# arcee-ai/DALM

Hardware: NVIDIA H100
Metric: RAG-e2e train-step samples/sec (bge-large + Llama-2-7B, bs=18) (higher is better)
Workload: dtype bf16

## Files before the change

dalm_b200/csrc/common.cuh:

```cuda
#pragma once
#include <cuda_runtime.h>
#include <cuda_bf16.h>
#include <stdint.h>
#include <stdio.h>
#include <string.h>

struct CUtensorMap_st;

namespace dalm {

void set_error(const char* fmt, ...);
int  check_launch(const char* what);
void count_launch(int n = 1);

#define DALM_REQUIRE(cond, ...)                                   \
  do {                                                            \
    if (!(cond)) { ::dalm::set_error(__VA_ARGS__); return 1; }    \
  } while (0)

#define DALM_CUDA(expr)                                                                   \
  do {                                                                                    \
    cudaError_t _e = (expr);                                                              \
    if (_e != cudaSuccess) {                                                              \
      ::dalm::set_error("%s failed: %s (%s:%d)", #expr, cudaGetErrorString(_e), __FILE__, \
                        __LINE__);                                                        \
      return 2;                                                                           \
    }                                                                                     \
  } while (0)

int num_sms();
long long l2_bytes();

int get_tmap(const void* ptr, long long rows, long long cols, long long ld, int box_rows, ::CUtensorMap_st* out, int f32 = 0);

__device__ __forceinline__ float warp_sum(float v) {
#pragma unroll
  for (int o = 16; o > 0; o >>= 1) v += __shfl_xor_sync(0xffffffffu, v, o);
  return v;
}
__device__ __forceinline__ float warp_max(float v) {
#pragma unroll
  for (int o = 16; o > 0; o >>= 1) v = fmaxf(v, __shfl_xor_sync(0xffffffffu, v, o));
  return v;
}
__device__ __forceinline__ double warp_sum_d(double v) {
#pragma unroll
  for (int o = 16; o > 0; o >>= 1) v += __shfl_xor_sync(0xffffffffu, v, o);
  return v;
}

__device__ __forceinline__ float block_sum(float v, float* red) {
  const int lane = threadIdx.x & 31, wid = threadIdx.x >> 5, nw = (blockDim.x + 31) >> 5;
  v = warp_sum(v);
  __syncthreads();
  if (lane == 0) red[wid] = v;
  __syncthreads();
  float r = (lane < nw) ? red[lane] : 0.f;
  r = warp_sum(r);
  return r;
}
__device__ __forceinline__ float block_max(float v, float* red) {
  const int lane = threadIdx.x & 31, wid = threadIdx.x >> 5, nw = (blockDim.x + 31) >> 5;
  v = warp_max(v);
  __syncthreads();
  if (lane == 0) red[wid] = v;
  __syncthreads();
  float r = (lane < nw) ? red[lane] : -INFINITY;
  r = warp_max(r);
  return r;
}

struct __align__(16) bf16x8 { __nv_bfloat162 v[4]; };

__device__ __forceinline__ void unpack8(const bf16x8& p, float* f) {
#pragma unroll
  for (int i = 0; i < 4; ++i) {
    float2 t = __bfloat1622float2(p.v[i]);
    f[2 * i] = t.x; f[2 * i + 1] = t.y;
  }
}
__device__ __forceinline__ bf16x8 pack8(const float* f) {
  bf16x8 p;
#pragma unroll
  for (int i = 0; i < 4; ++i) p.v[i] = __floats2bfloat162_rn(f[2 * i], f[2 * i + 1]);
  return p;
}

__device__ __forceinline__ float gelu_erf(float x) {
  return 0.5f * x * (1.f + erff(x * 0.70710678118654752440f));
}
__device__ __forceinline__ float gelu_erf_grad(float x) {
  const float cdf = 0.5f * (1.f + erff(x * 0.70710678118654752440f));
  const float pdf = 0.39894228040143267794f * __expf(-0.5f * x * x);
  return cdf + x * pdf;
}


struct DropCfg {
  float p;
  float inv_keep;
  unsigned int thresh;
  unsigned long long seed, stream;
  const unsigned long long* offset;
};
inline DropCfg make_drop(float p, unsigned long long seed, unsigned long long stream, const void* offset) {
  DropCfg d;
  d.p = p;
  double t = (double)p * 65536.0 + 0.5;
  d.thresh = p > 0.f ? (t >= 65535.0 ? 65535u : (unsigned int)t) : 0u;
  d.inv_keep = p > 0.f ? (float)(1.0 / (1.0 - (double)d.thresh / 65536.0)) : 1.f;
  d.seed = seed; d.stream = stream; d.offset = (const unsigned long long*)offset;
  return d;
}
__device__ __forceinline__ uint4 philox4x32_7(uint2 key, uint4 c) {
#pragma unroll
  for (int r = 0; r < 7; ++r) {
    const unsigned int hi0 = __umulhi(0xD2511F53u, c.x), lo0 = 0xD2511F53u * c.x;
    const unsigned int hi1 = __umulhi(0xCD9E8D57u, c.z), lo1 = 0xCD9E8D57u * c.z;
    c = make_uint4(hi1 ^ c.y ^ key.x, lo1, hi0 ^ c.w ^ key.y, lo0);
    key.x += 0x9E3779B9u; key.y += 0xBB67AE85u;
  }
  return c;
}
__device__ __forceinline__ unsigned long long drop_stream(const DropCfg& d) {
  return d.stream + (d.offset ? (*d.offset) * 0x9E3779B97F4A7C15ull : 0ull);
}
__device__ __forceinline__ void drop_scale8(const DropCfg& d, unsigned long long stream, unsigned long long idx8, float* scale) {
  const uint4 r = philox4x32_7(make_uint2((unsigned int)d.seed, (unsigned int)(d.seed >> 32)),
                               make_uint4((unsigned int)idx8, (unsigned int)(idx8 >> 32), (unsigned int)stream,
                                          (unsigned int)(stream >> 32)));
  const unsigned int w[4] = {r.x, r.y, r.z, r.w};
#pragma unroll
  for (int j = 0; j < 4; ++j) {
    scale[2 * j]     = (w[j] & 0xFFFFu) >= d.thresh ? d.inv_keep : 0.f;
    scale[2 * j + 1] = (w[j] >> 16)     >= d.thresh ? d.inv_keep : 0.f;
  }
}
__device__ __forceinline__ float drop_scale1(const DropCfg& d, unsigned long long stream, unsigned long long idx) {
  float sc[8];
  drop_scale8(d, stream, idx >> 3, sc);
  float v = sc[0];
#pragma unroll
  for (int j = 1; j < 8; ++j) if ((idx & 7) == (unsigned long long)j) v = sc[j];
  return v;
}

}
```

dalm_b200/csrc/gemm_wgmma.cu:

```cuda
#include "common.cuh"
#include "ptx.cuh"
#include <cudaTypedefs.h>
#include <mutex>
#include <unordered_map>

namespace dalm {
using namespace ptx;

enum class Epi {
  Plain,
  SwiGLU,
  RoPE,
  GeluPair,
  NormRoPE,
};

struct GemmEpilogue {
  void* out;
  long long ldo;
  int out_f32;
  const float* bias;
  const void* resid;
  long long ldr;
  int resid_f32;
  int act;
  float alpha;
  int M, N, K;
  DropCfg drop;
  int group_m;
  const float* rope_cos; const float* rope_sin;
  int rope_L, rope_cols;
  const float* q_norm; const float* k_norm;
  int nq_heads;
  float norm_eps;
  float* norm_rstd; long long ld_rstd;
  int norm_pre;
  int l2_hints;
};

__device__ __forceinline__ void tile_coords(int tile, int num_m, int num_n, int gm, int& m_blk, int& n_blk) {
  if (gm <= 0) { m_blk = tile % num_m; n_blk = tile / num_m; return; }
  const int band_tiles = gm * num_n;
  const int band = tile / band_tiles;
  const int r = tile - band * band_tiles;
  const int m0 = band * gm;
  const int h = min(gm, num_m - m0);
  const int n = r / h;
  m_blk = m0 + (r - n * h);
  n_blk = (band & 1) ? (num_n - 1 - n) : n;
}

template <bool PRE = false>
__device__ __forceinline__ void epilogue_math(const GemmEpilogue& ep, const uint32_t* v, float* f, int row, int col0, bool row_ok,
                                              const float4* rpre = nullptr) {
  const int N = ep.N;
#pragma unroll
  for (int i = 0; i < 32; ++i) f[i] = __uint_as_float(v[i]) * ep.alpha;
  if (ep.bias) {
#pragma unroll
    for (int i = 0; i < 32; ++i) if (col0 + i < N) f[i] += __ldg(ep.bias + col0 + i);
  }
  if (ep.act == 1) {
#pragma unroll
    for (int i = 0; i < 32; ++i) f[i] = gelu_erf(f[i]);
  }
  if (ep.drop.p > 0.f) {
    const unsigned long long dstream = drop_stream(ep.drop);
    const unsigned long long base = ((unsigned long long)row * (unsigned long long)N + (unsigned long long)col0) >> 3;
#pragma unroll
    for (int g = 0; g < 4; ++g) {
      float sc[8];
      drop_scale8(ep.drop, dstream, base + g, sc);
#pragma unroll
      for (int j = 0; j < 8; ++j) f[g * 8 + j] *= sc[j];
    }
  }
  if constexpr (PRE) {
#pragma unroll
    for (int g = 0; g < 8; ++g) { f[g * 4 + 0] += rpre[g].x; f[g * 4 + 1] += rpre[g].y; f[g * 4 + 2] += rpre[g].z; f[g * 4 + 3] += rpre[g].w; }
  } else if (ep.resid && row_ok) {
    if (ep.resid_f32) {
      const float* r = reinterpret_cast<const float*>(ep.resid) + (size_t)row * ep.ldr + col0;
#pragma unroll
      for (int g = 0; g < 8; ++g) {
        if (col0 + g * 4 < N) {
          const float4 t = *reinterpret_cast<const float4*>(r + g * 4);
          f[g * 4 + 0] += t.x; f[g * 4 + 1] += t.y; f[g * 4 + 2] += t.z; f[g * 4 + 3] += t.w;
        }
      }
    } else {
      const __nv_bfloat16* r = reinterpret_cast<const __nv_bfloat16*>(ep.resid) + (size_t)row * ep.ldr + col0;
#pragma unroll
      for (int g = 0; g < 4; ++g) {
        if (col0 + g * 8 < N) {
          const bf16x8 t = *reinterpret_cast<const bf16x8*>(r + g * 8);
          float tf[8];
          unpack8(t, tf);
          if (ep.act == 2) {
#pragma unroll
            for (int i = 0; i < 8; ++i) f[g * 8 + i] = __bfloat162float(__float2bfloat16_rn(f[g * 8 + i])) * gelu_erf_grad(tf[i]);
          } else {
#pragma unroll
            for (int i = 0; i < 8; ++i) f[g * 8 + i] += tf[i];
          }
        }
      }
    }
  }
}

__device__ __forceinline__ void acc_ld32(const float* p, uint32_t* v) {
#pragma unroll
  for (int g = 0; g < 8; ++g) {
    const float4 t = *reinterpret_cast<const float4*>(p + g * 4);
    v[g * 4 + 0] = __float_as_uint(t.x); v[g * 4 + 1] = __float_as_uint(t.y);
    v[g * 4 + 2] = __float_as_uint(t.z); v[g * 4 + 3] = __float_as_uint(t.w);
  }
}

constexpr int kStageTileBytes = 128 * 128;
constexpr int kEpiGroups = 2;
constexpr int kGemmThreads = 128 + kEpiGroups * 128;
template <int BN, Epi EPI>
__device__ __forceinline__ void epilogue_drain_tile(const GemmEpilogue& ep, const CUtensorMap* tmap_out, const CUtensorMap* tmap_out2,
                                                    unsigned char* staging, int grp, const float* arow, int row_in_tile, int tile_row0,
                                                    int tile_col0) {
  static_assert(BN == 256 || EPI == Epi::Plain || EPI == Epi::GeluPair, "the SwiGLU and RoPE epilogues need 256-wide tiles");
  const int N = ep.N;
  const int row = tile_row0 + row_in_tile;
  const bool row_ok = row < ep.M;
  constexpr bool F32_OUT = EPI == Epi::Plain;
  const int sb_cols = (F32_OUT && ep.out_f32) ? 32 : 64;
  const bool issuer = (threadIdx.x == 128 + grp * 128);
  unsigned char* tile = staging + grp * kStageTileBytes;
  unsigned char* st = tile + row_in_tile * 128;
  const int sw = row_in_tile & 7;
  const bool rpf = F32_OUT && ep.out_f32 && ep.resid != nullptr && ep.resid_f32;
  float4 rnext[8];
  auto fetch_resid = [&](int cc) {
    const int cg0 = tile_col0 + cc;
    const float* r = reinterpret_cast<const float*>(ep.resid) + (size_t)row * ep.ldr + cg0;
#pragma unroll
    for (int g = 0; g < 8; ++g)
      rnext[g] = (row_ok && cc < BN && cg0 + g * 4 < N) ? *reinterpret_cast<const float4*>(r + g * 4) : make_float4(0.f, 0.f, 0.f, 0.f);
  };
  if (rpf) fetch_resid(grp * sb_cols);
#pragma unroll 1
  for (int c = grp * sb_cols; c < BN; c += kEpiGroups * sb_cols) {
    const int col0 = tile_col0 + c;
    if (col0 >= N) break;
    if (issuer) bulk_wait_read<0>();
    named_bar_sync(1 + grp, 128);
    if (F32_OUT && ep.out_f32) {
      uint32_t v[32]; float f[32];
      acc_ld32(arow + c, v);
      if (rpf) {
        epilogue_math<true>(ep, v, f, row, col0, row_ok, rnext);
        fetch_resid(c + kEpiGroups * sb_cols);
      } else {
        epilogue_math<false>(ep, v, f, row, col0, row_ok);
      }
#pragma unroll
      for (int g = 0; g < 8; ++g)
        *reinterpret_cast<float4*>(st + ((g ^ sw) << 4)) = make_float4(f[g * 4], f[g * 4 + 1], f[g * 4 + 2], f[g * 4 + 3]);
    } else if (EPI == Epi::RoPE && col0 < ep.rope_cols) {
      const bool second = ((col0 >> 6) & 1) != 0;
      const int cp = second ? c - 64 : c + 64;
      const int colp = tile_col0 + cp;
      const int pos = row_ok ? (row % ep.rope_L) : 0;
      const float* cs = ep.rope_cos + (size_t)pos * 64;
      const float* sn = ep.rope_sin + (size_t)pos * 64;
#pragma unroll
      for (int h = 0; h < 2; ++h) {
        uint32_t vo[32], vq[32]; float f[32];
        acc_ld32(arow + (c + h * 32), vo);
        acc_ld32(arow + (cp + h * 32), vq);
        float cc[32], ss[32];
#pragma unroll
        for (int i = 0; i < 32; i += 4) {
          *reinterpret_cast<float4*>(cc + i) = __ldg(reinterpret_cast<const float4*>(cs + h * 32 + i));
          *reinterpret_cast<float4*>(ss + i) = __ldg(reinterpret_cast<const float4*>(sn + h * 32 + i));
        }
#pragma unroll
        for (int i = 0; i < 32; ++i) {
          float own = __uint_as_float(vo[i]), oth = __uint_as_float(vq[i]);
          if (ep.bias) {
            own += __ldg(ep.bias + col0 + h * 32 + i);
            oth += __ldg(ep.bias + colp + h * 32 + i);
          }
          f[i] = second ? fmaf(own, cc[i], oth * ss[i]) : fmaf(own, cc[i], -oth * ss[i]);
        }
#pragma unroll
        for (int g = 0; g < 4; ++g)
          *reinterpret_cast<bf16x8*>(st + (((h * 4 + g) ^ sw) << 4)) = pack8(f + g * 8);
      }
    } else if (EPI == Epi::NormRoPE && col0 < ep.rope_cols) {
      const bool second = ((col0 >> 6) & 1) != 0;
      const int cp = second ? c - 64 : c + 64;
      const int colp = tile_col0 + cp;
      const int c1 = second ? cp : c;
      const int head = col0 >> 7;
      const float* nw = head < ep.nq_heads ? ep.q_norm : ep.k_norm;
      const int jo = second ? 64 : 0, jp = 64 - jo;
      float ss = 0.f;
#pragma unroll 1
      for (int h = 0; h < 4; ++h) {
        uint32_t v[32];
        acc_ld32(arow + (c1 + h * 32), v);
#pragma unroll
        for (int i = 0; i < 32; ++i) {
          float x = __uint_as_float(v[i]);
          if (ep.bias) x += __ldg(ep.bias + tile_col0 + c1 + h * 32 + i);
          ss = fmaf(x, x, ss);
        }
      }
      const float rstd = rsqrtf(ss * (1.f / 128.f) + ep.norm_eps);
      if (ep.norm_rstd && row_ok && !second) ep.norm_rstd[(size_t)row * ep.ld_rstd + head] = rstd;
      const int pos = row_ok ? (row % ep.rope_L) : 0;
      const float* cs = ep.rope_cos + (size_t)pos * 64;
      const float* sn = ep.rope_sin + (size_t)pos * 64;
#pragma unroll
      for (int h = 0; h < 2; ++h) {
        uint32_t vo[32], vq[32]; float f[32];
        acc_ld32(arow + (c + h * 32), vo);
        acc_ld32(arow + (cp + h * 32), vq);
        float cc[32], ss2[32];
#pragma unroll
        for (int i = 0; i < 32; i += 4) {
          *reinterpret_cast<float4*>(cc + i) = __ldg(reinterpret_cast<const float4*>(cs + h * 32 + i));
          *reinterpret_cast<float4*>(ss2 + i) = __ldg(reinterpret_cast<const float4*>(sn + h * 32 + i));
        }
#pragma unroll
        for (int i = 0; i < 32; ++i) {
          float own = __uint_as_float(vo[i]), oth = __uint_as_float(vq[i]);
          if (ep.bias) {
            own += __ldg(ep.bias + col0 + h * 32 + i);
            oth += __ldg(ep.bias + colp + h * 32 + i);
          }
          own = own * rstd * __ldg(nw + jo + h * 32 + i);
          oth = oth * rstd * __ldg(nw + jp + h * 32 + i);
          f[i] = second ? fmaf(own, cc[i], oth * ss2[i]) : fmaf(own, cc[i], -oth * ss2[i]);
        }
#pragma unroll
        for (int g = 0; g < 4; ++g)
          *reinterpret_cast<bf16x8*>(st + (((h * 4 + g) ^ sw) << 4)) = pack8(f + g * 8);
      }
      fence_proxy_async();
      named_bar_sync(1 + grp, 128);
      if (issuer) {
        if (ep.l2_hints & 4) tma_store_2d_hint(tmap_out, tile, col0, tile_row0, l2_policy_evict_first());
        else                 tma_store_2d(tmap_out, tile, col0, tile_row0);
        bulk_commit();
      }
      if (!ep.norm_pre) continue;
      if (issuer) bulk_wait_read<0>();
      named_bar_sync(1 + grp, 128);
#pragma unroll
      for (int h = 0; h < 2; ++h) {
        uint32_t v[32]; float f[32];
        acc_ld32(arow + (c + h * 32), v);
#pragma unroll
        for (int i = 0; i < 32; ++i) {
          f[i] = __uint_as_float(v[i]);
          if (ep.bias) f[i] += __ldg(ep.bias + col0 + h * 32 + i);
        }
#pragma unroll
        for (int g = 0; g < 4; ++g)
          *reinterpret_cast<bf16x8*>(st + (((h * 4 + g) ^ sw) << 4)) = pack8(f + g * 8);
      }
      fence_proxy_async();
      named_bar_sync(1 + grp, 128);
      if (issuer) {
        tma_store_2d(tmap_out2, tile, col0, tile_row0);
        bulk_commit();
      }
      continue;
    } else if (EPI == Epi::GeluPair) {
      bf16x8 pk[8];
#pragma unroll
      for (int h = 0; h < 2; ++h) {
        if (col0 + h * 32 < N) {
          uint32_t v[32]; float f[32];
          acc_ld32(arow + (c + h * 32), v);
          epilogue_math(ep, v, f, row, col0 + h * 32, row_ok);
#pragma unroll
          for (int g = 0; g < 4; ++g) pk[h * 4 + g] = pack8(f + g * 8);
        } else {
#pragma unroll
          for (int g = 0; g < 4; ++g) pk[h * 4 + g] = bf16x8{};
        }
      }
#pragma unroll
      for (int g = 0; g < 8; ++g) *reinterpret_cast<bf16x8*>(st + ((g ^ sw) << 4)) = pk[g];
      fence_proxy_async();
      named_bar_sync(1 + grp, 128);
      if (issuer) {
        if (ep.l2_hints & 4) tma_store_2d_hint(tmap_out, tile, col0, tile_row0, l2_policy_evict_first());
        else                 tma_store_2d(tmap_out, tile, col0, tile_row0);
        bulk_commit();
      }
#pragma unroll
      for (int g = 0; g < 8; ++g) {
        float x[8];
        unpack8(pk[g], x);
#pragma unroll
        for (int i = 0; i < 8; ++i) x[i] = gelu_erf(x[i]);
        pk[g] = pack8(x);
      }
      if (issuer) bulk_wait_read<0>();
      named_bar_sync(1 + grp, 128);
#pragma unroll
      for (int g = 0; g < 8; ++g) *reinterpret_cast<bf16x8*>(st + ((g ^ sw) << 4)) = pk[g];
      fence_proxy_async();
      named_bar_sync(1 + grp, 128);
      if (issuer) {
        tma_store_2d(tmap_out2, tile, col0, tile_row0);
        bulk_commit();
      }
      continue;
    } else {
#pragma unroll
      for (int h = 0; h < 2; ++h) {
        if (col0 + h * 32 < N) {
          uint32_t v[32]; float f[32];
          acc_ld32(arow + (c + h * 32), v);
          epilogue_math(ep, v, f, row, col0 + h * 32, row_ok);
#pragma unroll
          for (int g = 0; g < 4; ++g)
            *reinterpret_cast<bf16x8*>(st + (((h * 4 + g) ^ sw) << 4)) = pack8(f + g * 8);
        }
      }
    }
    fence_proxy_async();
    named_bar_sync(1 + grp, 128);
    if (issuer) {
      if (ep.l2_hints & 4) tma_store_2d_hint(tmap_out, tile, col0, tile_row0, l2_policy_evict_first());
      else                 tma_store_2d(tmap_out, tile, col0, tile_row0);
      bulk_commit();
    }
  }
  if constexpr (EPI == Epi::SwiGLU) {
    const int j = grp;
    const int acol0 = (tile_col0 >> 1) + j * 64;
    if (issuer) bulk_wait_read<0>();
    named_bar_sync(1 + grp, 128);
#pragma unroll
    for (int h = 0; h < 2; ++h) {
      uint32_t vg[32], vu[32]; float f[32];
      acc_ld32(arow + (j * 64 + h * 32), vg);
      acc_ld32(arow + (128 + j * 64 + h * 32), vu);
#pragma unroll
      for (int i = 0; i < 32; ++i) {
        const float g = __uint_as_float(vg[i]);
        f[i] = g / (1.f + __expf(-g)) * __uint_as_float(vu[i]);
      }
#pragma unroll
      for (int g4 = 0; g4 < 4; ++g4) *reinterpret_cast<bf16x8*>(st + (((h * 4 + g4) ^ sw) << 4)) = pack8(f + g4 * 8);
    }
    fence_proxy_async();
    named_bar_sync(1 + grp, 128);
    if (issuer) {
      if (ep.l2_hints & 4) tma_store_2d_hint(tmap_out2, tile, acol0, tile_row0, l2_policy_evict_first());
      else                 tma_store_2d(tmap_out2, tile, acol0, tile_row0);
      bulk_commit();
    }
  }
}

template <int BN> struct GemmCfg {
  static constexpr int BM = 128, BK = 64;
  static constexpr int A_BYTES = BM * BK * 2;
  static constexpr int B_BYTES = BN * BK * 2;
  static constexpr int STAGE_BYTES = A_BYTES + B_BYTES;
  static constexpr int STAGES = (BN == 256) ? 4 : (BN == 128 ? 6 : 8);
  static constexpr int ACC_LD = BN + 4;
  static constexpr int SMEM_BYTES = STAGES * STAGE_BYTES + 2 * kStageTileBytes + 1024  + 256 ;
  static_assert(BM * ACC_LD * 4 <= STAGES * STAGE_BYTES, "the accumulator tile reuses the stage ring");
  static_assert(SMEM_BYTES <= 232448, "exceeds 227 KB of shared memory per block");
};

template <int BN, int TA, int TB>
__device__ __forceinline__ void wgmma_tile(float* d, uint64_t da, uint64_t db, int scale_d) {
  if constexpr (BN == 256) wgmma_m64n256k16<TA, TB>(d, da, db, scale_d);
  else if constexpr (BN == 128) wgmma_m64n128k16<TA, TB>(d, da, db, scale_d);
  else wgmma_m64n64k16<TA, TB>(d, da, db, scale_d);
}

template <int BN, int LAYOUT, Epi EPI, int CL>
__global__ void __launch_bounds__(kGemmThreads, 1)
gemm_bf16_tn_kernel(const __grid_constant__ CUtensorMap tmap_a, const __grid_constant__ CUtensorMap tmap_b,
                    const __grid_constant__ CUtensorMap tmap_out, const __grid_constant__ CUtensorMap tmap_out2, const GemmEpilogue ep) {
  using Cfg = GemmCfg<BN>;
  constexpr int BM = Cfg::BM, BK = Cfg::BK, STAGES = Cfg::STAGES;
  static_assert(CL == 1 || (LAYOUT == 0 && EPI == Epi::Plain), "the cluster kernel takes the plain TN layout");
  extern __shared__ unsigned char smem_raw[];
  unsigned char* smem = reinterpret_cast<unsigned char*>((reinterpret_cast<uintptr_t>(smem_raw) + 1023) & ~uintptr_t(1023));
  unsigned char* staging = smem + STAGES * Cfg::STAGE_BYTES;
  uint64_t* full_bar  = reinterpret_cast<uint64_t*>(staging + 2 * kStageTileBytes);
  uint64_t* empty_bar = full_bar + STAGES;
  uint64_t* epi_bar   = empty_bar + STAGES;
  float* acc_smem = reinterpret_cast<float*>(smem);

  const int warp = threadIdx.x >> 5, lane = threadIdx.x & 31;
  const uint32_t rank = CL == 2 ? cluster_ctarank() : 0u;
  const int M = ep.M, N = ep.N, K = ep.K;
  const int num_m = (M + CL * BM - 1) / (CL * BM), num_n = (N + BN - 1) / BN;
  const int num_tiles = num_m * num_n;
  const int num_kb = (K + BK - 1) / BK;
  const int unit = blockIdx.x / CL, num_units = gridDim.x / CL;
  const int group_m = CL == 2 ? 0 : ep.group_m;

  if (threadIdx.x == 0) {
    prefetch_tmap(&tmap_a);
    prefetch_tmap(&tmap_b);
    prefetch_tmap(&tmap_out);
    if constexpr (EPI == Epi::SwiGLU || EPI == Epi::GeluPair || EPI == Epi::NormRoPE) prefetch_tmap(&tmap_out2);
  }
  if (threadIdx.x == 32) {
    for (int s = 0; s < STAGES; ++s) { mbar_init(&full_bar[s], 1); mbar_init(&empty_bar[s], 8 * CL); }
    mbar_init(epi_bar, 8 * CL);
    fence_mbar_init();
  }
  if constexpr (CL == 2) cluster_sync_all();
  else __syncthreads();

  if (warp < 4) {
    asm volatile("setmaxnreg.dec.sync.aligned.u32 40;" ::: "memory");
    if (warp == 0 && lane == 0) {
      int stage = 0; uint32_t phase = 0;
      const bool hint_a = (ep.l2_hints & 1) != 0, hint_b = (ep.l2_hints & 2) != 0;
      const uint64_t pol_a = hint_a ? l2_policy_evict_last() : 0ull, pol_b = hint_b ? l2_policy_evict_first() : 0ull;
      auto load = [](void* dst, const CUtensorMap* tm, uint64_t* bar, int c0, int c1, bool hinted, uint64_t pol) {
        if (hinted) tma_load_2d_hint(dst, tm, bar, c0, c1, pol);
        else        tma_load_2d(dst, tm, bar, c0, c1);
      };
      int it = 0;
      for (int tile = unit; tile < num_tiles; tile += num_units, ++it) {
        int m_blk, n_blk;
        tile_coords(tile, num_m, num_n, group_m, m_blk, n_blk);
        if (it > 0) mbar_wait(epi_bar, (uint32_t)(it - 1) & 1u);
        for (int kb = 0; kb < num_kb; ++kb) {
          mbar_wait(&empty_bar[stage], phase ^ 1);
          unsigned char* sa = smem + stage * Cfg::STAGE_BYTES;
          unsigned char* sb = sa + Cfg::A_BYTES;
          mbar_arrive_expect_tx(&full_bar[stage], Cfg::STAGE_BYTES);
          if constexpr (CL == 2) {
            load(sa, &tmap_a, &full_bar[stage], kb * BK, (m_blk * CL + (int)rank) * BM, hint_a, pol_a);
            tma_load_2d_multicast(sb + rank * (Cfg::B_BYTES / 2), &tmap_b, &full_bar[stage], kb * BK, n_blk * BN + (int)rank * (BN / 2), 0x3);
          } else {
            if constexpr (LAYOUT == 2) {
#pragma unroll
              for (int c = 0; c < BM / 64; ++c) load(sa + c * 8192, &tmap_a, &full_bar[stage], m_blk * BM + c * 64, kb * BK, hint_a, pol_a);
            } else {
              load(sa, &tmap_a, &full_bar[stage], kb * BK, m_blk * BM, hint_a, pol_a);
            }
            if constexpr (LAYOUT >= 1) {
#pragma unroll
              for (int c = 0; c < BN / 64; ++c) load(sb + c * 8192, &tmap_b, &full_bar[stage], n_blk * BN + c * 64, kb * BK, hint_b, pol_b);
            } else {
              load(sb, &tmap_b, &full_bar[stage], kb * BK, n_blk * BN, hint_b, pol_b);
            }
          }
          if (++stage == STAGES) { stage = 0; phase ^= 1; }
        }
      }
    }
  } else {
    asm volatile("setmaxnreg.inc.sync.aligned.u32 232;" ::: "memory");
    const int grp = (warp - 4) >> 2;
    const int q = warp & 3;
    constexpr int TA = LAYOUT == 2 ? 1 : 0, TB = LAYOUT >= 1 ? 1 : 0;
    constexpr uint64_t a_step = TA ? 128 : 2, b_step = TB ? 128 : 2;
    const uint32_t a_off = (uint32_t)grp * 8192u;
    int stage = 0; uint32_t phase = 0;
    for (int tile = unit; tile < num_tiles; tile += num_units) {
      int m_blk, n_blk;
      tile_coords(tile, num_m, num_n, group_m, m_blk, n_blk);
      float acc[BN / 2];
      int prev = -1;
      for (int kb = 0; kb < num_kb; ++kb) {
        mbar_wait(&full_bar[stage], phase);
        const uint32_t sa = smem_u32(smem + stage * Cfg::STAGE_BYTES);
        const uint32_t sb = sa + Cfg::A_BYTES;
        const uint64_t adesc = TA ? make_sw128_mnmajor_desc(sa + a_off, 8192, 1024) : make_sw128_kmajor_desc(sa + a_off);
        const uint64_t bdesc = TB ? make_sw128_mnmajor_desc(sb, 8192, 1024) : make_sw128_kmajor_desc(sb);
        wgmma_fence();
#pragma unroll
        for (int k = 0; k < BK / 16; ++k)
          wgmma_tile<BN, TA, TB>(acc, adesc + a_step * (uint64_t)k, bdesc + b_step * (uint64_t)k, (kb | k) != 0 ? 1 : 0);
        wgmma_commit();
        wgmma_wait<1>();
        if (prev >= 0 && lane == 0) {
          mbar_arrive(&empty_bar[prev]);
          if constexpr (CL == 2) mbar_arrive_remote(&empty_bar[prev], rank ^ 1u);
        }
        prev = stage;
        if (++stage == STAGES) { stage = 0; phase ^= 1; }
      }
      wgmma_wait<0>();
      if (lane == 0) {
        mbar_arrive(&empty_bar[prev]);
        if constexpr (CL == 2) mbar_arrive_remote(&empty_bar[prev], rank ^ 1u);
      }
      named_bar_sync(3, 256);
      {
        const int r0 = grp * 64 + q * 16 + (lane >> 2);
        float* p0 = acc_smem + (size_t)r0 * Cfg::ACC_LD + 2 * (lane & 3);
        float* p1 = p0 + 8 * Cfg::ACC_LD;
#pragma unroll
        for (int j = 0; j < BN / 8; ++j) {
          *reinterpret_cast<float2*>(p0 + 8 * j) = make_float2(acc[4 * j], acc[4 * j + 1]);
          *reinterpret_cast<float2*>(p1 + 8 * j) = make_float2(acc[4 * j + 2], acc[4 * j + 3]);
        }
      }
      named_bar_sync(3, 256);
      const int row_in_tile = q * 32 + lane;
      epilogue_drain_tile<BN, EPI>(ep, &tmap_out, &tmap_out2, staging, grp, acc_smem + (size_t)row_in_tile * Cfg::ACC_LD,
                                   row_in_tile, (m_blk * CL + (int)rank) * BM, n_blk * BN);
      fence_proxy_async();
      __syncwarp();
      if (lane == 0) {
        mbar_arrive(epi_bar);
        if constexpr (CL == 2) mbar_arrive_remote(epi_bar, rank ^ 1u);
      }
    }
    if ((threadIdx.x & 127) == 0) bulk_wait<0>();
  }
  if constexpr (CL == 2) cluster_sync_all();
}

static PFN_cuTensorMapEncodeTiled_v12000 get_encode_fn() {
  static PFN_cuTensorMapEncodeTiled_v12000 fn = nullptr;
  static std::once_flag once;
  std::call_once(once, [] {
    void* p = nullptr;
    cudaDriverEntryPointQueryResult qres;
    if (cudaGetDriverEntryPoint("cuTensorMapEncodeTiled", &p, cudaEnableDefault, &qres) == cudaSuccess &&
        qres == cudaDriverEntryPointSuccess)
      fn = reinterpret_cast<PFN_cuTensorMapEncodeTiled_v12000>(p);
  });
  return fn;
}

struct TmapKey {
  const void* ptr; long long rows, cols, ld; int box_rows; int f32;
  bool operator==(const TmapKey& o) const {
    return ptr == o.ptr && rows == o.rows && cols == o.cols && ld == o.ld && box_rows == o.box_rows && f32 == o.f32;
  }
};
struct TmapKeyHash {
  size_t operator()(const TmapKey& k) const {
    size_t h = reinterpret_cast<size_t>(k.ptr);
    h = h * 1000003u ^ (size_t)k.rows; h = h * 1000003u ^ (size_t)k.cols;
    h = h * 1000003u ^ (size_t)k.ld;   h = h * 1000003u ^ (size_t)(k.box_rows * 2 + k.f32);
    return h;
  }
};
static std::unordered_map<TmapKey, CUtensorMap, TmapKeyHash> g_tmaps;
static std::mutex g_tmap_mu;

int get_tmap(const void* ptr, long long rows, long long cols, long long ld, int box_rows, CUtensorMap* out, int f32) {
  TmapKey key{ptr, rows, cols, ld, box_rows, f32};
  {
    std::lock_guard<std::mutex> g(g_tmap_mu);
    auto it = g_tmaps.find(key);
    if (it != g_tmaps.end()) { *out = it->second; return 0; }
  }
  auto fn = get_encode_fn();
  DALM_REQUIRE(fn != nullptr, "gemm: cuTensorMapEncodeTiled driver entry point unavailable");
  DALM_REQUIRE((reinterpret_cast<uintptr_t>(ptr) & 15) == 0, "gemm: operand base %p is not 16-byte aligned", ptr);
  DALM_REQUIRE((ld % (f32 ? 4 : 8)) == 0, "gemm: row stride %lld is not a multiple of 16 bytes", ld);
  cuuint64_t dims[2] = {(cuuint64_t)cols, (cuuint64_t)rows};
  cuuint64_t strides[1] = {(cuuint64_t)ld * (f32 ? 4 : 2)};
  cuuint32_t box[2] = {f32 ? 32u : 64u, (cuuint32_t)box_rows};
  cuuint32_t estr[2] = {1u, 1u};
  CUtensorMap m;
  CUresult r = fn(&m, f32 ? CU_TENSOR_MAP_DATA_TYPE_FLOAT32 : CU_TENSOR_MAP_DATA_TYPE_BFLOAT16, 2, const_cast<void*>(ptr), dims, strides, box, estr,
                  CU_TENSOR_MAP_INTERLEAVE_NONE, CU_TENSOR_MAP_SWIZZLE_128B, CU_TENSOR_MAP_L2_PROMOTION_L2_256B,
                  CU_TENSOR_MAP_FLOAT_OOB_FILL_NONE);
  DALM_REQUIRE(r == CUDA_SUCCESS, "gemm: cuTensorMapEncodeTiled failed (%d) rows=%lld cols=%lld ld=%lld box_rows=%d",
               (int)r, rows, cols, ld, box_rows);
  {
    std::lock_guard<std::mutex> g(g_tmap_mu);
    if (g_tmaps.size() > 8192) g_tmaps.clear();
    g_tmaps[key] = m;
  }
  *out = m;
  return 0;
}

template <int BN, int LAYOUT, Epi EPI>
static int launch_gemm(const CUtensorMap& ta, const CUtensorMap& tb, const CUtensorMap& to, const GemmEpilogue& ep,
                       int max_ctas, cudaStream_t stream, const CUtensorMap* to2) {
  using Cfg = GemmCfg<BN>;
  static bool attr_set = false;
  if (!attr_set) {
    DALM_CUDA(cudaFuncSetAttribute(gemm_bf16_tn_kernel<BN, LAYOUT, EPI, 1>, cudaFuncAttributeMaxDynamicSharedMemorySize, Cfg::SMEM_BYTES));
    attr_set = true;
  }
  const int num_tiles = ((ep.M + 127) / 128) * ((ep.N + BN - 1) / BN);
  int grid = num_tiles < num_sms() ? num_tiles : num_sms();
  if (max_ctas > 0 && grid > max_ctas) grid = max_ctas;
  gemm_bf16_tn_kernel<BN, LAYOUT, EPI, 1><<<grid, kGemmThreads, Cfg::SMEM_BYTES, stream>>>(ta, tb, to, to2 ? *to2 : to, ep);
  count_launch();
  return check_launch("gemm_bf16_tn_kernel");
}

template <int LAYOUT, Epi EPI>
static int launch_gemm_bn(int bn, const CUtensorMap& ta, const CUtensorMap& tb, const CUtensorMap& to, const GemmEpilogue& ep,
                          int max_ctas, cudaStream_t stream, const CUtensorMap* to2 = nullptr) {
  if (bn == 256) return launch_gemm<256, LAYOUT, EPI>(ta, tb, to, ep, max_ctas, stream, to2);
  if (bn == 128) return launch_gemm<128, LAYOUT, EPI>(ta, tb, to, ep, max_ctas, stream, to2);
  return launch_gemm<64, LAYOUT, EPI>(ta, tb, to, ep, max_ctas, stream, to2);
}

template <int BN>
static int launch_gemm_cluster(const CUtensorMap& ta, const CUtensorMap& tb, const CUtensorMap& to, const GemmEpilogue& ep,
                               int max_ctas, cudaStream_t stream) {
  using Cfg = GemmCfg<BN>;
  auto kern = gemm_bf16_tn_kernel<BN, 0, Epi::Plain, 2>;
  static bool attr_set = false;
  if (!attr_set) {
    DALM_CUDA(cudaFuncSetAttribute(kern, cudaFuncAttributeMaxDynamicSharedMemorySize, Cfg::SMEM_BYTES));
    attr_set = true;
  }
  const int num_tiles = ((ep.M + 255) / 256) * ((ep.N + BN - 1) / BN);
  int clusters = num_tiles < num_sms() / 2 ? num_tiles : num_sms() / 2;
  if (max_ctas > 0 && clusters > max_ctas / 2) clusters = max_ctas / 2 > 0 ? max_ctas / 2 : 1;
  cudaLaunchConfig_t cfg = {};
  cfg.gridDim = dim3(2 * clusters);
  cfg.blockDim = dim3(kGemmThreads);
  cfg.dynamicSmemBytes = Cfg::SMEM_BYTES;
  cfg.stream = stream;
  cudaLaunchAttribute attr[1];
  attr[0].id = cudaLaunchAttributeClusterDimension;
  attr[0].val.clusterDim.x = 2; attr[0].val.clusterDim.y = 1; attr[0].val.clusterDim.z = 1;
  cfg.attrs = attr; cfg.numAttrs = 1;
  DALM_CUDA(cudaLaunchKernelEx(&cfg, kern, ta, tb, to, to, ep));
  count_launch();
  return check_launch("gemm_bf16_tn_kernel (cluster of 2)");
}

}

using namespace dalm;

static int env_int(const char* name, int dflt) {
  const char* v = getenv(name);
  return (v && *v) ? atoi(v) : dflt;
}
static int g_group_m_override = env_int("DALM_B200_GEMM_RASTER", 0);
extern "C" void dalm_b200_gemm_set_raster(int group_m) { g_group_m_override = group_m; }
static int g_l2_hints = env_int("DALM_B200_GEMM_L2_HINTS", -1);
static double l2_resident_a() { return (double)l2_bytes() / 3.0; }
extern "C" void dalm_b200_gemm_set_l2_hints(int mask) { g_l2_hints = mask < 0 ? -1 : (mask & 7); }
static int pick_l2_hints(int M, int N, int K, int tile_n, int group_m, bool stream_out) {
  if (g_l2_hints >= 0) return g_l2_hints;
  const long long tiles = (long long)((M + 127) / 128) * ((N + tile_n - 1) / tile_n);
  return (group_m == 0 && tiles > num_sms() && 2.0 * M * K <= l2_resident_a() && !stream_out) ? 7 : 0;
}

static int pick_block_n(int M, int N) {
  const long long m1 = (M + 127) / 128;
  double best = 1e30;
  int bn = 64;
  const int cand[3] = {256, 128, 64};
  const double penalty[3] = {1.0, 1.55, 2.7};
  for (int i = 0; i < 3; ++i) {
    if (cand[i] > 64 && N < cand[i]) continue;
    const long long tiles = m1 * ((N + cand[i] - 1) / cand[i]);
    const double cost = (double)((tiles + num_sms() - 1) / num_sms()) * cand[i] * penalty[i];
    if (cost < best) { best = cost; bn = cand[i]; }
  }
  return bn;
}

static int pick_group_m(int M, int N, int K, int tile_n, bool stream_out) {
  const int num_m = (M + 127) / 128, num_n = (N + tile_n - 1) / tile_n;
  int group_m = 0;
  if (g_group_m_override > 0) return g_group_m_override;
  if (g_group_m_override == -1 || (long long)num_m * num_n <= num_sms()) return 0;
  const double a_bytes = 2.0 * M * K;
  if (g_group_m_override == 0 && a_bytes <= l2_resident_a() && !stream_out) return 0;
  const double ideal = sqrt((double)num_sms() * tile_n / 128.0);
  int nbands = (int)(num_m / ideal + 0.5);
  if (nbands < 1) nbands = 1;
  group_m = (num_m + nbands - 1) / nbands;
  if (group_m >= num_m) group_m = 0;
  return group_m;
}

static GemmEpilogue gemm_epilogue(int M, int N, int K, int tile_n, void* out, long long ldo, int out_f32 = 0,
                                  const void* resid = nullptr, long long ldr = 0, int resid_f32 = 0) {
  GemmEpilogue ep{};
  ep.out = out; ep.ldo = ldo; ep.out_f32 = out_f32;
  ep.resid = resid; ep.ldr = ldr; ep.resid_f32 = resid_f32;
  ep.alpha = 1.f;
  ep.M = M; ep.N = N; ep.K = K;
  ep.drop = make_drop(0.f, 0, 0, nullptr);
  const bool stream_out = out_f32 != 0 || resid != nullptr;
  ep.group_m = pick_group_m(M, N, K, tile_n, stream_out);
  ep.l2_hints = pick_l2_hints(M, N, K, tile_n, ep.group_m, stream_out);
  return ep;
}

extern "C" int dalm_b200_gemm_bf16(int layout, const void* A, long long lda, const void* B, long long ldb, void* out,
                                   long long ldo, int out_f32, int M, int N, int K, float alpha, const float* bias,
                                   int act, const void* resid, long long ldr, int resid_f32, int block_n,
                                   int max_ctas, float drop_p, unsigned long long drop_seed,
                                   unsigned long long drop_stream_id, const void* drop_offset, void* stream) {
  DALM_REQUIRE(layout >= 0 && layout <= 2, "gemm: layout must be 0 (TN), 1 (NN) or 2 (wgrad)");
  DALM_REQUIRE(M > 0 && N > 0 && K > 0, "gemm: empty problem M=%d N=%d K=%d", M, N, K);
  DALM_REQUIRE((N % 8) == 0, "gemm: N=%d must be a multiple of 8", N);
  DALM_REQUIRE((K % 8) == 0 || layout == 2, "gemm: K=%d must be a multiple of 8", K);
  DALM_REQUIRE((M % 8) == 0 || layout != 2, "gemm: M=%d must be a multiple of 8 for the wgrad layout", M);
  DALM_REQUIRE(lda >= (layout == 2 ? M : K) && ldb >= (layout >= 1 ? N : K) && ldo >= N, "gemm: leading dimensions too small");
  DALM_REQUIRE((ldo % (out_f32 ? 4 : 8)) == 0, "gemm: ldo=%lld breaks 16-byte row alignment", ldo);
  DALM_REQUIRE((reinterpret_cast<uintptr_t>(out) & 15) == 0, "gemm: out is not 16-byte aligned");
  if (resid) {
    DALM_REQUIRE((ldr % (resid_f32 ? 4 : 8)) == 0, "gemm: ldr=%lld breaks 16-byte row alignment", ldr);
    DALM_REQUIRE((reinterpret_cast<uintptr_t>(resid) & 15) == 0, "gemm: resid is not 16-byte aligned");
  }
  DALM_REQUIRE(act == 0 || act == 1 || act == 2, "gemm: act must be 0 (none), 1 (gelu) or 2 (gelu backward: multiply by gelu'(resid))");
  DALM_REQUIRE(act != 2 || (resid != nullptr && !resid_f32 && !out_f32 && drop_p == 0.f),
               "gemm: act 2 (gelu backward) needs a bf16 `resid` (the pre-activation), a bf16 output and no dropout");
  int bn = block_n;
  if (bn == 0) bn = pick_block_n(M, N);
  DALM_REQUIRE(bn == 64 || bn == 128 || bn == 256 || bn == 2128 || bn == 2256,
               "gemm: block_n must be 0, 64/128/256 (single CTA) or 2128/2256 (cluster of two CTAs)");
  const bool pair = bn > 1000;
  DALM_REQUIRE(!(pair && layout != 0), "gemm: the cluster kernel only takes the TN layout");
  const int tile_n = pair ? bn % 1000 : bn;
  CUtensorMap ta, tb, to;
  if (layout == 2) { if (int e = get_tmap(A, K, M, lda, 64, &ta)) return e; }
  else             { if (int e = get_tmap(A, M, K, lda, 128, &ta)) return e; }
  if (layout >= 1) { if (int e = get_tmap(B, K, N, ldb, 64, &tb)) return e; }
  else             { if (int e = get_tmap(B, N, K, ldb, pair ? tile_n / 2 : tile_n, &tb)) return e; }
  if (int e = get_tmap(out, M, N, ldo, 128, &to, out_f32)) return e;
  DALM_REQUIRE(drop_p >= 0.f && drop_p < 1.f, "gemm: dropout p must be in [0,1)");
  GemmEpilogue ep = gemm_epilogue(M, N, K, tile_n, out, ldo, out_f32, resid, ldr, resid_f32);
  ep.bias = bias; ep.act = act; ep.alpha = alpha;
  ep.drop = make_drop(drop_p, drop_seed, drop_stream_id, drop_offset);
  cudaStream_t st = (cudaStream_t)stream;
  if (bn == 2256) return launch_gemm_cluster<256>(ta, tb, to, ep, max_ctas, st);
  if (bn == 2128) return launch_gemm_cluster<128>(ta, tb, to, ep, max_ctas, st);
  if (layout == 1) return launch_gemm_bn<1, Epi::Plain>(bn, ta, tb, to, ep, max_ctas, st);
  if (layout == 2) return launch_gemm_bn<2, Epi::Plain>(bn, ta, tb, to, ep, max_ctas, st);
  return launch_gemm_bn<0, Epi::Plain>(bn, ta, tb, to, ep, max_ctas, st);
}

extern "C" int dalm_b200_gemm_bf16_swiglu(const void* A, long long lda, const void* B, long long ldb, void* gu, long long ldgu,
                                          void* act, long long ldact, int M, int N, int K, void* stream) {
  DALM_REQUIRE(M > 0 && K > 0 && N >= 256 && (N % 256) == 0, "gemm_swiglu: N=%d must be a positive multiple of 256 (128-feature gate / up blocks)", N);
  DALM_REQUIRE((K % 8) == 0 && lda >= K && ldb >= K && ldgu >= N && ldact >= N / 2, "gemm_swiglu: bad K / leading dimensions");
  DALM_REQUIRE((ldgu % 8) == 0 && (ldact % 8) == 0 && ((uintptr_t)gu & 15) == 0 && ((uintptr_t)act & 15) == 0, "gemm_swiglu: output alignment");
  CUtensorMap ta, tb, to, to2;
  if (int e = get_tmap(A, M, K, lda, 128, &ta)) return e;
  if (int e = get_tmap(B, N, K, ldb, 256, &tb)) return e;
  if (int e = get_tmap(gu, M, N, ldgu, 128, &to, 0)) return e;
  if (int e = get_tmap(act, M, N / 2, ldact, 128, &to2, 0)) return e;
  const GemmEpilogue ep = gemm_epilogue(M, N, K, 256, gu, ldgu);
  return launch_gemm<256, 0, Epi::SwiGLU>(ta, tb, to, ep, 0, (cudaStream_t)stream, &to2);
}

extern "C" int dalm_b200_gemm_bf16_gelu(const void* A, long long lda, const void* B, long long ldb, void* pre, long long ldpre,
                                        void* act, long long ldact, int M, int N, int K, const float* bias, void* stream) {
  DALM_REQUIRE(M > 0 && N > 0 && K > 0 && (N % 8) == 0 && (K % 8) == 0, "gemm_gelu: bad shape M=%d N=%d K=%d", M, N, K);
  DALM_REQUIRE(lda >= K && ldb >= K && ldpre >= N && ldact >= N, "gemm_gelu: leading dimensions too small");
  DALM_REQUIRE((ldpre % 8) == 0 && (ldact % 8) == 0 && ((uintptr_t)pre & 15) == 0 && ((uintptr_t)act & 15) == 0, "gemm_gelu: output alignment");
  const int bn = pick_block_n(M, N);
  CUtensorMap ta, tb, to, to2;
  if (int e = get_tmap(A, M, K, lda, 128, &ta)) return e;
  if (int e = get_tmap(B, N, K, ldb, bn, &tb)) return e;
  if (int e = get_tmap(pre, M, N, ldpre, 128, &to, 0)) return e;
  if (int e = get_tmap(act, M, N, ldact, 128, &to2, 0)) return e;
  GemmEpilogue ep = gemm_epilogue(M, N, K, bn, pre, ldpre);
  ep.bias = bias;
  return launch_gemm_bn<0, Epi::GeluPair>(bn, ta, tb, to, ep, 0, (cudaStream_t)stream, &to2);
}

extern "C" int dalm_b200_gemm_bf16_rope(const void* A, long long lda, const void* B, long long ldb, void* out, long long ldo, int M,
                                        int N, int K, const float* bias, const float* cos_t, const float* sin_t, int L, int rope_cols,
                                        const float* q_norm, const float* k_norm, int nq_heads, float eps, void* pre_out,
                                        long long ld_pre, float* rstd_out, long long ld_rstd, void* stream) {
  DALM_REQUIRE(M > 0 && N > 0 && K > 0 && (N % 8) == 0 && (K % 8) == 0, "gemm_rope: bad shape M=%d N=%d K=%d", M, N, K);
  DALM_REQUIRE(rope_cols > 0 && rope_cols <= N && (rope_cols % 256) == 0, "gemm_rope: rope_cols=%d must be a multiple of 256 (whole 128-wide heads per tile)", rope_cols);
  DALM_REQUIRE(L > 0 && cos_t != nullptr && sin_t != nullptr && ((uintptr_t)cos_t & 15) == 0 && ((uintptr_t)sin_t & 15) == 0, "gemm_rope: cos / sin tables");
  DALM_REQUIRE(lda >= K && ldb >= K && ldo >= N && (ldo % 8) == 0 && ((uintptr_t)out & 15) == 0, "gemm_rope: leading dimensions / alignment");
  CUtensorMap ta, tb, to;
  if (int e = get_tmap(A, M, K, lda, 128, &ta)) return e;
  if (int e = get_tmap(B, N, K, ldb, 256, &tb)) return e;
  if (int e = get_tmap(out, M, N, ldo, 128, &to, 0)) return e;
  GemmEpilogue ep = gemm_epilogue(M, N, K, 256, out, ldo);
  ep.bias = bias;
  ep.rope_cos = cos_t; ep.rope_sin = sin_t; ep.rope_L = L; ep.rope_cols = rope_cols;
  if (q_norm == nullptr) {
    DALM_REQUIRE(k_norm == nullptr && pre_out == nullptr && rstd_out == nullptr, "gemm_rope: k_norm / pre_out / rstd_out need q_norm");
    return launch_gemm<256, 0, Epi::RoPE>(ta, tb, to, ep, 0, (cudaStream_t)stream, nullptr);
  }
  DALM_REQUIRE(k_norm != nullptr && nq_heads >= 0 && nq_heads <= rope_cols / 128 && eps >= 0.f, "gemm_rope: norm weights / nq_heads=%d", nq_heads);
  DALM_REQUIRE(rstd_out == nullptr || ld_rstd >= rope_cols / 128, "gemm_rope: ld_rstd=%lld < %d heads", ld_rstd, rope_cols / 128);
  CUtensorMap to2 = to;
  if (pre_out != nullptr) {
    DALM_REQUIRE(ld_pre >= rope_cols && (ld_pre % 8) == 0 && ((uintptr_t)pre_out & 15) == 0, "gemm_rope: pre_out leading dimension / alignment");
    if (int e = get_tmap(pre_out, M, rope_cols, ld_pre, 128, &to2, 0)) return e;
  }
  ep.q_norm = q_norm; ep.k_norm = k_norm; ep.nq_heads = nq_heads; ep.norm_eps = eps;
  ep.norm_rstd = rstd_out; ep.ld_rstd = ld_rstd; ep.norm_pre = pre_out != nullptr;
  return launch_gemm<256, 0, Epi::NormRoPE>(ta, tb, to, ep, 0, (cudaStream_t)stream, &to2);
}

extern "C" void dalm_b200_gemm_clear_cache() {
  std::lock_guard<std::mutex> g(g_tmap_mu);
  g_tmaps.clear();
}
```

Measured before the change: 70.65.

## Run GEMM epilogue directly from registers and drop the smem accumulator round-trip

```diff
diff --git a/dalm_b200/csrc/common.cuh b/dalm_b200/csrc/common.cuh
--- a/dalm_b200/csrc/common.cuh
+++ b/dalm_b200/csrc/common.cuh
@@ -125,10 +125,12 @@
 __device__ __forceinline__ unsigned long long drop_stream(const DropCfg& d) {
   return d.stream + (d.offset ? (*d.offset) * 0x9E3779B97F4A7C15ull : 0ull);
 }
+__device__ __forceinline__ uint4 drop_bits8(const DropCfg& d, unsigned long long stream, unsigned long long idx8) {
+  return philox4x32_7(make_uint2((unsigned int)d.seed, (unsigned int)(d.seed >> 32)),
+                      make_uint4((unsigned int)idx8, (unsigned int)(idx8 >> 32), (unsigned int)stream, (unsigned int)(stream >> 32)));
+}
 __device__ __forceinline__ void drop_scale8(const DropCfg& d, unsigned long long stream, unsigned long long idx8, float* scale) {
-  const uint4 r = philox4x32_7(make_uint2((unsigned int)d.seed, (unsigned int)(d.seed >> 32)),
-                               make_uint4((unsigned int)idx8, (unsigned int)(idx8 >> 32), (unsigned int)stream,
-                                          (unsigned int)(stream >> 32)));
+  const uint4 r = drop_bits8(d, stream, idx8);
   const unsigned int w[4] = {r.x, r.y, r.z, r.w};
 #pragma unroll
   for (int j = 0; j < 4; ++j) {
diff --git a/dalm_b200/csrc/gemm_wgmma.cu b/dalm_b200/csrc/gemm_wgmma.cu
--- a/dalm_b200/csrc/gemm_wgmma.cu
+++ b/dalm_b200/csrc/gemm_wgmma.cu
@@ -50,58 +50,100 @@
   n_blk = (band & 1) ? (num_n - 1 - n) : n;
 }
 
-template <bool PRE = false>
-__device__ __forceinline__ void epilogue_math(const GemmEpilogue& ep, const uint32_t* v, float* f, int row, int col0, bool row_ok,
-                                              const float4* rpre = nullptr) {
+constexpr int kBoxRows = 64;
+constexpr int kBoxBytes = kBoxRows * 128;
+constexpr int kStageTileBytes = 2 * kBoxBytes;
+constexpr int kEpiGroups = 2;
+constexpr int kGemmThreads = 128 + kEpiGroups * 128;
+
+struct EpiStage {
+  unsigned char* boxes;
+  int bar;
+  bool issuer;
+  int buf;
+  __device__ __forceinline__ unsigned char* begin() {
+    if (issuer) bulk_wait_read<1>();
+    named_bar_sync(bar, 128);
+    return boxes + buf * kBoxBytes;
+  }
+  __device__ __forceinline__ void end(const CUtensorMap* tm, int col, int row, bool evict_first) {
+    fence_proxy_async();
+    named_bar_sync(bar, 128);
+    if (issuer) {
+      const unsigned char* box = boxes + buf * kBoxBytes;
+      if (evict_first) tma_store_2d_hint(tm, box, col, row, l2_policy_evict_first());
+      else             tma_store_2d(tm, box, col, row);
+      bulk_commit();
+    }
+    buf ^= 1;
+  }
+};
+
+__device__ __forceinline__ void box_st_bf16x2(unsigned char* box, int r, int b, float lo, float hi) {
+  *reinterpret_cast<__nv_bfloat162*>(box + r * 128 + ((((b >> 4) ^ (r & 7)) << 4) | (b & 15))) = __floats2bfloat162_rn(lo, hi);
+}
+__device__ __forceinline__ void box_st_f32x2(unsigned char* box, int r, int b, float lo, float hi) {
+  *reinterpret_cast<float2*>(box + r * 128 + ((((b >> 4) ^ (r & 7)) << 4) | (b & 15))) = make_float2(lo, hi);
+}
+
+__device__ __forceinline__ void epilogue_math(const GemmEpilogue& ep, float* x, int row, int col, bool ok0, bool ok1,
+                                              unsigned long long dstream, bool resid_loaded = false) {
   const int N = ep.N;
 #pragma unroll
-  for (int i = 0; i < 32; ++i) f[i] = __uint_as_float(v[i]) * ep.alpha;
+  for (int i = 0; i < 8; ++i) x[i] *= ep.alpha;
   if (ep.bias) {
 #pragma unroll
-    for (int i = 0; i < 32; ++i) if (col0 + i < N) f[i] += __ldg(ep.bias + col0 + i);
+    for (int jj = 0; jj < 2; ++jj) {
+      if (col + 8 * jj < N) {
+        const float b0 = __ldg(ep.bias + col + 8 * jj), b1 = __ldg(ep.bias + col + 8 * jj + 1);
+        x[4 * jj + 0] += b0; x[4 * jj + 1] += b1; x[4 * jj + 2] += b0; x[4 * jj + 3] += b1;
+      }
+    }
   }
   if (ep.act == 1) {
 #pragma unroll
-    for (int i = 0; i < 32; ++i) f[i] = gelu_erf(f[i]);
+    for (int i = 0; i < 8; ++i) x[i] = gelu_erf(x[i]);
   }
   if (ep.drop.p > 0.f) {
-    const unsigned long long dstream = drop_stream(ep.drop);
-    const unsigned long long base = ((unsigned long long)row * (unsigned long long)N + (unsigned long long)col0) >> 3;
+    const int k = threadIdx.x & 3;
+    const unsigned long long idx8 = ((unsigned long long)(row + 8 * (k & 1)) * (unsigned long long)N +
+                                     (unsigned long long)(col - 2 * k + 8 * (k >> 1))) >> 3;
+    const uint4 r = drop_bits8(ep.drop, dstream, idx8);
+    unsigned int m0 = 0u, m1 = 0u, m2 = 0u, m3 = 0u;
+#pragma unroll
+    for (int s = 0; s < 4; ++s) {
+      const int t = k ^ s;
+      const unsigned int v = t == 0 ? r.x : t == 1 ? r.y : t == 2 ? r.z : r.w;
+      const unsigned int got = s ? __shfl_xor_sync(0xffffffffu, v, s) : v;
+      m0 = t == 0 ? got : m0; m1 = t == 1 ? got : m1; m2 = t == 2 ? got : m2; m3 = t == 3 ? got : m3;
+    }
+    const unsigned int m[4] = {m0, m1, m2, m3};
 #pragma unroll
     for (int g = 0; g < 4; ++g) {
-      float sc[8];
-      drop_scale8(ep.drop, dstream, base + g, sc);
-#pragma unroll
-      for (int j = 0; j < 8; ++j) f[g * 8 + j] *= sc[j];
-    }
-  }
-  if constexpr (PRE) {
-#pragma unroll
-    for (int g = 0; g < 8; ++g) { f[g * 4 + 0] += rpre[g].x; f[g * 4 + 1] += rpre[g].y; f[g * 4 + 2] += rpre[g].z; f[g * 4 + 3] += rpre[g].w; }
-  } else if (ep.resid && row_ok) {
-    if (ep.resid_f32) {
-      const float* r = reinterpret_cast<const float*>(ep.resid) + (size_t)row * ep.ldr + col0;
-#pragma unroll
-      for (int g = 0; g < 8; ++g) {
-        if (col0 + g * 4 < N) {
-          const float4 t = *reinterpret_cast<const float4*>(r + g * 4);
-          f[g * 4 + 0] += t.x; f[g * 4 + 1] += t.y; f[g * 4 + 2] += t.z; f[g * 4 + 3] += t.w;
-        }
-      }
-    } else {
-      const __nv_bfloat16* r = reinterpret_cast<const __nv_bfloat16*>(ep.resid) + (size_t)row * ep.ldr + col0;
-#pragma unroll
-      for (int g = 0; g < 4; ++g) {
-        if (col0 + g * 8 < N) {
-          const bf16x8 t = *reinterpret_cast<const bf16x8*>(r + g * 8);
-          float tf[8];
-          unpack8(t, tf);
+      x[2 * g + 0] *= (m[g] & 0xFFFFu) >= ep.drop.thresh ? ep.drop.inv_keep : 0.f;
+      x[2 * g + 1] *= (m[g] >> 16) >= ep.drop.thresh ? ep.drop.inv_keep : 0.f;
+    }
+  }
+  if (ep.resid && !resid_loaded) {
+#pragma unroll
+    for (int h = 0; h < 2; ++h) {
+      if (!(h ? ok1 : ok0)) continue;
+      const size_t roff = (size_t)(row + 8 * h) * ep.ldr;
+#pragma unroll
+      for (int jj = 0; jj < 2; ++jj) {
+        const int c = col + 8 * jj;
+        if (c >= N) continue;
+        float* v = x + 4 * jj + 2 * h;
+        if (ep.resid_f32) {
+          const float2 t = *reinterpret_cast<const float2*>(reinterpret_cast<const float*>(ep.resid) + roff + c);
+          v[0] += t.x; v[1] += t.y;
+        } else {
+          const float2 t = __bfloat1622float2(*reinterpret_cast<const __nv_bfloat162*>(reinterpret_cast<const __nv_bfloat16*>(ep.resid) + roff + c));
           if (ep.act == 2) {
-#pragma unroll
-            for (int i = 0; i < 8; ++i) f[g * 8 + i] = __bfloat162float(__float2bfloat16_rn(f[g * 8 + i])) * gelu_erf_grad(tf[i]);
+            v[0] = __bfloat162float(__float2bfloat16_rn(v[0])) * gelu_erf_grad(t.x);
+            v[1] = __bfloat162float(__float2bfloat16_rn(v[1])) * gelu_erf_grad(t.y);
           } else {
-#pragma unroll
-            for (int i = 0; i < 8; ++i) f[g * 8 + i] += tf[i];
+            v[0] += t.x; v[1] += t.y;
           }
         }
       }
@@ -109,261 +151,204 @@
   }
 }
 
-__device__ __forceinline__ void acc_ld32(const float* p, uint32_t* v) {
-#pragma unroll
-  for (int g = 0; g < 8; ++g) {
-    const float4 t = *reinterpret_cast<const float4*>(p + g * 4);
-    v[g * 4 + 0] = __float_as_uint(t.x); v[g * 4 + 1] = __float_as_uint(t.y);
-    v[g * 4 + 2] = __float_as_uint(t.z); v[g * 4 + 3] = __float_as_uint(t.w);
-  }
-}
-
-constexpr int kStageTileBytes = 128 * 128;
-constexpr int kEpiGroups = 2;
-constexpr int kGemmThreads = 128 + kEpiGroups * 128;
 template <int BN, Epi EPI>
-__device__ __forceinline__ void epilogue_drain_tile(const GemmEpilogue& ep, const CUtensorMap* tmap_out, const CUtensorMap* tmap_out2,
-                                                    unsigned char* staging, int grp, const float* arow, int row_in_tile, int tile_row0,
-                                                    int tile_col0) {
+__device__ __forceinline__ void epilogue_tile(const GemmEpilogue& ep, const CUtensorMap* tmap_out, const CUtensorMap* tmap_out2,
+                                              EpiStage& sg, float (&acc)[BN / 2], int row0, int tile_col0) {
   static_assert(BN == 256 || EPI == Epi::Plain || EPI == Epi::GeluPair, "the SwiGLU and RoPE epilogues need 256-wide tiles");
   const int N = ep.N;
-  const int row = tile_row0 + row_in_tile;
-  const bool row_ok = row < ep.M;
-  constexpr bool F32_OUT = EPI == Epi::Plain;
-  const int sb_cols = (F32_OUT && ep.out_f32) ? 32 : 64;
-  const bool issuer = (threadIdx.x == 128 + grp * 128);
-  unsigned char* tile = staging + grp * kStageTileBytes;
-  unsigned char* st = tile + row_in_tile * 128;
-  const int sw = row_in_tile & 7;
-  const bool rpf = F32_OUT && ep.out_f32 && ep.resid != nullptr && ep.resid_f32;
-  float4 rnext[8];
-  auto fetch_resid = [&](int cc) {
-    const int cg0 = tile_col0 + cc;
-    const float* r = reinterpret_cast<const float*>(ep.resid) + (size_t)row * ep.ldr + cg0;
-#pragma unroll
-    for (int g = 0; g < 8; ++g)
-      rnext[g] = (row_ok && cc < BN && cg0 + g * 4 < N) ? *reinterpret_cast<const float4*>(r + g * 4) : make_float4(0.f, 0.f, 0.f, 0.f);
+  const int lane = threadIdx.x & 31, k = lane & 3;
+  const int rb = 16 * ((threadIdx.x >> 5) & 3) + (lane >> 2);
+  const int row = row0 + rb;
+  const bool ok0 = row < ep.M, ok1 = row + 8 < ep.M;
+  const int cq = tile_col0 + 2 * k;
+  const bool hint = (ep.l2_hints & 4) != 0;
+  const unsigned long long dstream = ep.drop.p > 0.f ? drop_stream(ep.drop) : 0ull;
+  auto frag8 = [&](float* x, int j0) {
+#pragma unroll
+    for (int i = 0; i < 8; ++i) x[i] = acc[4 * j0 + i];
   };
-  if (rpf) fetch_resid(grp * sb_cols);
+  auto shift8 = [&]() {
+#pragma unroll
+    for (int i = 0; i + 32 < BN / 2; ++i) acc[i] = acc[i + 32];
+  };
+
+  if (EPI == Epi::Plain && ep.out_f32) {
+    const bool rpf = ep.resid != nullptr && ep.resid_f32;
+    float2 rn[8];
+    auto fetch_resid = [&](int c) {
+#pragma unroll
+      for (int i = 0; i < 8; ++i) {
+        const int h = i & 1, cc = cq + c + 8 * (i >> 1);
+        rn[i] = ((h ? ok1 : ok0) && c < BN && cc < N)
+                    ? *reinterpret_cast<const float2*>(reinterpret_cast<const float*>(ep.resid) + (size_t)(row + 8 * h) * ep.ldr + cc)
+                    : make_float2(0.f, 0.f);
+      }
+    };
+    if (rpf) fetch_resid(0);
 #pragma unroll 1
-  for (int c = grp * sb_cols; c < BN; c += kEpiGroups * sb_cols) {
+    for (int c = 0; c < BN && tile_col0 + c < N; c += 64) {
+#pragma unroll
+      for (int b = 0; b < 2; ++b) {
+        const int cb = c + 32 * b;
+        if (tile_col0 + cb >= N) break;
+        unsigned char* box = sg.begin();
+#pragma unroll
+        for (int u = 0; u < 2; ++u) {
+          float x[8];
+          frag8(x, 4 * b + 2 * u);
+          epilogue_math(ep, x, row, cq + cb + 16 * u, ok0, ok1, dstream, rpf);
+#pragma unroll
+          for (int i = 0; i < 4; ++i) {
+            if (rpf) { x[2 * i] += rn[4 * u + i].x; x[2 * i + 1] += rn[4 * u + i].y; }
+          }
+#pragma unroll
+          for (int i = 0; i < 4; ++i) box_st_f32x2(box, rb + 8 * (i & 1), 64 * u + 32 * (i >> 1) + 8 * k, x[2 * i], x[2 * i + 1]);
+        }
+        if (rpf) fetch_resid(cb + 32);
+        sg.end(tmap_out, tile_col0 + cb, row0, hint);
+      }
+      shift8();
+    }
+    return;
+  }
+
+  if constexpr (EPI == Epi::SwiGLU) {
+#pragma unroll
+    for (int b = 0; b < 2; ++b) {
+      unsigned char* box = sg.begin();
+#pragma unroll
+      for (int jl = 0; jl < 8; ++jl) {
+        const int j = 8 * b + jl;
+#pragma unroll
+        for (int h = 0; h < 2; ++h) {
+          float f[2];
+#pragma unroll
+          for (int e = 0; e < 2; ++e) {
+            const float g = acc[4 * j + 2 * h + e];
+            f[e] = g / (1.f + __expf(-g)) * acc[4 * (j + 16) + 2 * h + e];
+          }
+          box_st_bf16x2(box, rb + 8 * h, 16 * jl + 4 * k, f[0], f[1]);
+        }
+      }
+      sg.end(tmap_out2, (tile_col0 >> 1) + 64 * b, row0, hint);
+    }
+  }
+  const bool rope_tile = (EPI == Epi::RoPE || EPI == Epi::NormRoPE) && tile_col0 < ep.rope_cols;
+  float rstd[2][2];
+  const float* nwt[2];
+  if (EPI == Epi::NormRoPE && rope_tile) {
+#pragma unroll
+    for (int hd = 0; hd < 2; ++hd) {
+      const int head = (tile_col0 >> 7) + hd;
+      nwt[hd] = head < ep.nq_heads ? ep.q_norm : ep.k_norm;
+#pragma unroll
+      for (int h = 0; h < 2; ++h) {
+        float ss = 0.f;
+#pragma unroll
+        for (int jl = 0; jl < 16; ++jl) {
+          const int j = 16 * hd + jl;
+#pragma unroll
+          for (int e = 0; e < 2; ++e) {
+            float x = acc[4 * j + 2 * h + e];
+            if (ep.bias) x += __ldg(ep.bias + cq + 8 * j + e);
+            ss = fmaf(x, x, ss);
+          }
+        }
+        ss += __shfl_xor_sync(0xffffffffu, ss, 1);
+        ss += __shfl_xor_sync(0xffffffffu, ss, 2);
+        rstd[hd][h] = rsqrtf(ss * (1.f / 128.f) + ep.norm_eps);
+        if (ep.norm_rstd && (h ? ok1 : ok0) && k == 0) ep.norm_rstd[(size_t)(row + 8 * h) * ep.ld_rstd + head] = rstd[hd][h];
+      }
+    }
+  }
+  if ((EPI == Epi::RoPE || EPI == Epi::NormRoPE) && rope_tile) {
+#pragma unroll
+    for (int c = 0; c < BN; c += 64) {
+      const int col0 = tile_col0 + c;
+      const int jb = c / 8;
+      const bool second = ((c >> 6) & 1) != 0;
+      const int jp = second ? -8 : 8;
+      const int hd = c >> 7;
+      const int io = (c & 64) + 2 * k, ip = ((c & 64) ^ 64) + 2 * k;
+      unsigned char* box = sg.begin();
+#pragma unroll
+      for (int h = 0; h < 2; ++h) {
+        const int pos = (h ? ok1 : ok0) ? (row + 8 * h) % ep.rope_L : 0;
+        const float* cs = ep.rope_cos + (size_t)pos * 64 + 2 * k;
+        const float* sn = ep.rope_sin + (size_t)pos * 64 + 2 * k;
+#pragma unroll
+        for (int jl = 0; jl < 8; ++jl) {
+          const int j = jb + jl;
+          const float2 cc = __ldg(reinterpret_cast<const float2*>(cs + 8 * jl));
+          const float2 s2 = __ldg(reinterpret_cast<const float2*>(sn + 8 * jl));
+          float f[2];
+#pragma unroll
+          for (int e = 0; e < 2; ++e) {
+            float own = acc[4 * j + 2 * h + e], oth = acc[4 * (j + jp) + 2 * h + e];
+            if (ep.bias) {
+              own += __ldg(ep.bias + cq + 8 * j + e);
+              oth += __ldg(ep.bias + cq + 8 * (j + jp) + e);
+            }
+            if constexpr (EPI == Epi::NormRoPE) {
+              own = own * rstd[hd][h] * __ldg(nwt[hd] + io + 8 * jl + e);
+              oth = oth * rstd[hd][h] * __ldg(nwt[hd] + ip + 8 * jl + e);
+            }
+            const float cv = e ? cc.y : cc.x, sv = e ? s2.y : s2.x;
+            f[e] = second ? fmaf(own, cv, oth * sv) : fmaf(own, cv, -oth * sv);
+          }
+          box_st_bf16x2(box, rb + 8 * h, 16 * jl + 4 * k, f[0], f[1]);
+        }
+      }
+      sg.end(tmap_out, col0, row0, hint);
+      if (EPI == Epi::NormRoPE && ep.norm_pre) {
+        box = sg.begin();
+#pragma unroll
+        for (int jl = 0; jl < 8; ++jl) {
+          const int j = jb + jl;
+#pragma unroll
+          for (int h = 0; h < 2; ++h) {
+            float f[2];
+#pragma unroll
+            for (int e = 0; e < 2; ++e) {
+              f[e] = acc[4 * j + 2 * h + e];
+              if (ep.bias) f[e] += __ldg(ep.bias + cq + 8 * j + e);
+            }
+            box_st_bf16x2(box, rb + 8 * h, 16 * jl + 4 * k, f[0], f[1]);
+          }
+        }
+        sg.end(tmap_out2, col0, row0, false);
+      }
+    }
+    return;
+  }
+#pragma unroll 1
+  for (int c = 0; c < BN && tile_col0 + c < N; c += 64) {
     const int col0 = tile_col0 + c;
-    if (col0 >= N) break;
-    if (issuer) bulk_wait_read<0>();
-    named_bar_sync(1 + grp, 128);
-    if (F32_OUT && ep.out_f32) {
-      uint32_t v[32]; float f[32];
-      acc_ld32(arow + c, v);
-      if (rpf) {
-        epilogue_math<true>(ep, v, f, row, col0, row_ok, rnext);
-        fetch_resid(c + kEpiGroups * sb_cols);
-      } else {
-        epilogue_math<false>(ep, v, f, row, col0, row_ok);
-      }
-#pragma unroll
-      for (int g = 0; g < 8; ++g)
-        *reinterpret_cast<float4*>(st + ((g ^ sw) << 4)) = make_float4(f[g * 4], f[g * 4 + 1], f[g * 4 + 2], f[g * 4 + 3]);
-    } else if (EPI == Epi::RoPE && col0 < ep.rope_cols) {
-      const bool second = ((col0 >> 6) & 1) != 0;
-      const int cp = second ? c - 64 : c + 64;
-      const int colp = tile_col0 + cp;
-      const int pos = row_ok ? (row % ep.rope_L) : 0;
-      const float* cs = ep.rope_cos + (size_t)pos * 64;
-      const float* sn = ep.rope_sin + (size_t)pos * 64;
-#pragma unroll
-      for (int h = 0; h < 2; ++h) {
-        uint32_t vo[32], vq[32]; float f[32];
-        acc_ld32(arow + (c + h * 32), vo);
-        acc_ld32(arow + (cp + h * 32), vq);
-        float cc[32], ss[32];
-#pragma unroll
-        for (int i = 0; i < 32; i += 4) {
-          *reinterpret_cast<float4*>(cc + i) = __ldg(reinterpret_cast<const float4*>(cs + h * 32 + i));
-          *reinterpret_cast<float4*>(ss + i) = __ldg(reinterpret_cast<const float4*>(sn + h * 32 + i));
-        }
-#pragma unroll
-        for (int i = 0; i < 32; ++i) {
-          float own = __uint_as_float(vo[i]), oth = __uint_as_float(vq[i]);
-          if (ep.bias) {
-            own += __ldg(ep.bias + col0 + h * 32 + i);
-            oth += __ldg(ep.bias + colp + h * 32 + i);
-          }
-          f[i] = second ? fmaf(own, cc[i], oth * ss[i]) : fmaf(own, cc[i], -oth * ss[i]);
-        }
-#pragma unroll
-        for (int g = 0; g < 4; ++g)
-          *reinterpret_cast<bf16x8*>(st + (((h * 4 + g) ^ sw) << 4)) = pack8(f + g * 8);
-      }
-    } else if (EPI == Epi::NormRoPE && col0 < ep.rope_cols) {
-      const bool second = ((col0 >> 6) & 1) != 0;
-      const int cp = second ? c - 64 : c + 64;
-      const int colp = tile_col0 + cp;
-      const int c1 = second ? cp : c;
-      const int head = col0 >> 7;
-      const float* nw = head < ep.nq_heads ? ep.q_norm : ep.k_norm;
-      const int jo = second ? 64 : 0, jp = 64 - jo;
-      float ss = 0.f;
-#pragma unroll 1
-      for (int h = 0; h < 4; ++h) {
-        uint32_t v[32];
-        acc_ld32(arow + (c1 + h * 32), v);
-#pragma unroll
-        for (int i = 0; i < 32; ++i) {
-          float x = __uint_as_float(v[i]);
-          if (ep.bias) x += __ldg(ep.bias + tile_col0 + c1 + h * 32 + i);
-          ss = fmaf(x, x, ss);
-        }
-      }
-      const float rstd = rsqrtf(ss * (1.f / 128.f) + ep.norm_eps);
-      if (ep.norm_rstd && row_ok && !second) ep.norm_rstd[(size_t)row * ep.ld_rstd + head] = rstd;
-      const int pos = row_ok ? (row % ep.rope_L) : 0;
-      const float* cs = ep.rope_cos + (size_t)pos * 64;
-      const float* sn = ep.rope_sin + (size_t)pos * 64;
-#pragma unroll
-      for (int h = 0; h < 2; ++h) {
-        uint32_t vo[32], vq[32]; float f[32];
-        acc_ld32(arow + (c + h * 32), vo);
-        acc_ld32(arow + (cp + h * 32), vq);
-        float cc[32], ss2[32];
-#pragma unroll
-        for (int i = 0; i < 32; i += 4) {
-          *reinterpret_cast<float4*>(cc + i) = __ldg(reinterpret_cast<const float4*>(cs + h * 32 + i));
-          *reinterpret_cast<float4*>(ss2 + i) = __ldg(reinterpret_cast<const float4*>(sn + h * 32 + i));
-        }
-#pragma unroll
-        for (int i = 0; i < 32; ++i) {
-          float own = __uint_as_float(vo[i]), oth = __uint_as_float(vq[i]);
-          if (ep.bias) {
-            own += __ldg(ep.bias + col0 + h * 32 + i);
-            oth += __ldg(ep.bias + colp + h * 32 + i);
-          }
-          own = own * rstd * __ldg(nw + jo + h * 32 + i);
-          oth = oth * rstd * __ldg(nw + jp + h * 32 + i);
-          f[i] = second ? fmaf(own, cc[i], oth * ss2[i]) : fmaf(own, cc[i], -oth * ss2[i]);
-        }
-#pragma unroll
-        for (int g = 0; g < 4; ++g)
-          *reinterpret_cast<bf16x8*>(st + (((h * 4 + g) ^ sw) << 4)) = pack8(f + g * 8);
-      }
-      fence_proxy_async();
-      named_bar_sync(1 + grp, 128);
-      if (issuer) {
-        if (ep.l2_hints & 4) tma_store_2d_hint(tmap_out, tile, col0, tile_row0, l2_policy_evict_first());
-        else                 tma_store_2d(tmap_out, tile, col0, tile_row0);
-        bulk_commit();
-      }
-      if (!ep.norm_pre) continue;
-      if (issuer) bulk_wait_read<0>();
-      named_bar_sync(1 + grp, 128);
-#pragma unroll
-      for (int h = 0; h < 2; ++h) {
-        uint32_t v[32]; float f[32];
-        acc_ld32(arow + (c + h * 32), v);
-#pragma unroll
-        for (int i = 0; i < 32; ++i) {
-          f[i] = __uint_as_float(v[i]);
-          if (ep.bias) f[i] += __ldg(ep.bias + col0 + h * 32 + i);
-        }
-#pragma unroll
-        for (int g = 0; g < 4; ++g)
-          *reinterpret_cast<bf16x8*>(st + (((h * 4 + g) ^ sw) << 4)) = pack8(f + g * 8);
-      }
-      fence_proxy_async();
-      named_bar_sync(1 + grp, 128);
-      if (issuer) {
-        tma_store_2d(tmap_out2, tile, col0, tile_row0);
-        bulk_commit();
-      }
-      continue;
-    } else if (EPI == Epi::GeluPair) {
-      bf16x8 pk[8];
-#pragma unroll
-      for (int h = 0; h < 2; ++h) {
-        if (col0 + h * 32 < N) {
-          uint32_t v[32]; float f[32];
-          acc_ld32(arow + (c + h * 32), v);
-          epilogue_math(ep, v, f, row, col0 + h * 32, row_ok);
-#pragma unroll
-          for (int g = 0; g < 4; ++g) pk[h * 4 + g] = pack8(f + g * 8);
-        } else {
-#pragma unroll
-          for (int g = 0; g < 4; ++g) pk[h * 4 + g] = bf16x8{};
-        }
-      }
-#pragma unroll
-      for (int g = 0; g < 8; ++g) *reinterpret_cast<bf16x8*>(st + ((g ^ sw) << 4)) = pk[g];
-      fence_proxy_async();
-      named_bar_sync(1 + grp, 128);
-      if (issuer) {
-        if (ep.l2_hints & 4) tma_store_2d_hint(tmap_out, tile, col0, tile_row0, l2_policy_evict_first());
-        else                 tma_store_2d(tmap_out, tile, col0, tile_row0);
-        bulk_commit();
-      }
-#pragma unroll
-      for (int g = 0; g < 8; ++g) {
-        float x[8];
-        unpack8(pk[g], x);
-#pragma unroll
-        for (int i = 0; i < 8; ++i) x[i] = gelu_erf(x[i]);
-        pk[g] = pack8(x);
-      }
-      if (issuer) bulk_wait_read<0>();
-      named_bar_sync(1 + grp, 128);
-#pragma unroll
-      for (int g = 0; g < 8; ++g) *reinterpret_cast<bf16x8*>(st + ((g ^ sw) << 4)) = pk[g];
-      fence_proxy_async();
-      named_bar_sync(1 + grp, 128);
-      if (issuer) {
-        tma_store_2d(tmap_out2, tile, col0, tile_row0);
-        bulk_commit();
-      }
-      continue;
-    } else {
-#pragma unroll
-      for (int h = 0; h < 2; ++h) {
-        if (col0 + h * 32 < N) {
-          uint32_t v[32]; float f[32];
-          acc_ld32(arow + (c + h * 32), v);
-          epilogue_math(ep, v, f, row, col0 + h * 32, row_ok);
-#pragma unroll
-          for (int g = 0; g < 4; ++g)
-            *reinterpret_cast<bf16x8*>(st + (((h * 4 + g) ^ sw) << 4)) = pack8(f + g * 8);
-        }
-      }
-    }
-    fence_proxy_async();
-    named_bar_sync(1 + grp, 128);
-    if (issuer) {
-      if (ep.l2_hints & 4) tma_store_2d_hint(tmap_out, tile, col0, tile_row0, l2_policy_evict_first());
-      else                 tma_store_2d(tmap_out, tile, col0, tile_row0);
-      bulk_commit();
-    }
-  }
-  if constexpr (EPI == Epi::SwiGLU) {
-    const int j = grp;
-    const int acol0 = (tile_col0 >> 1) + j * 64;
-    if (issuer) bulk_wait_read<0>();
-    named_bar_sync(1 + grp, 128);
-#pragma unroll
-    for (int h = 0; h < 2; ++h) {
-      uint32_t vg[32], vu[32]; float f[32];
-      acc_ld32(arow + (j * 64 + h * 32), vg);
-      acc_ld32(arow + (128 + j * 64 + h * 32), vu);
-#pragma unroll
-      for (int i = 0; i < 32; ++i) {
-        const float g = __uint_as_float(vg[i]);
-        f[i] = g / (1.f + __expf(-g)) * __uint_as_float(vu[i]);
-      }
-#pragma unroll
-      for (int g4 = 0; g4 < 4; ++g4) *reinterpret_cast<bf16x8*>(st + (((h * 4 + g4) ^ sw) << 4)) = pack8(f + g4 * 8);
-    }
-    fence_proxy_async();
-    named_bar_sync(1 + grp, 128);
-    if (issuer) {
-      if (ep.l2_hints & 4) tma_store_2d_hint(tmap_out2, tile, acol0, tile_row0, l2_policy_evict_first());
-      else                 tma_store_2d(tmap_out2, tile, acol0, tile_row0);
-      bulk_commit();
-    }
+    __nv_bfloat162 pk[16];
+    unsigned char* box = sg.begin();
+#pragma unroll
+    for (int u = 0; u < 4; ++u) {
+      float x[8];
+      frag8(x, 2 * u);
+      epilogue_math(ep, x, row, cq + c + 16 * u, ok0, ok1, dstream);
+#pragma unroll
+      for (int i = 0; i < 4; ++i) {
+        pk[4 * u + i] = __floats2bfloat162_rn(x[2 * i], x[2 * i + 1]);
+        *reinterpret_cast<__nv_bfloat162*>(box + (rb + 8 * (i & 1)) * 128 +
+                                           ((((2 * u + (i >> 1)) ^ (rb & 7)) << 4) | (4 * k))) = pk[4 * u + i];
+      }
+    }
+    sg.end(tmap_out, col0, row0, hint);
+    if constexpr (EPI == Epi::GeluPair) {
+      box = sg.begin();
+#pragma unroll
+      for (int i = 0; i < 16; ++i) {
+        const float2 p = __bfloat1622float2(pk[i]);
+        box_st_bf16x2(box, rb + 8 * (i & 1), 16 * (i >> 1) + 4 * k, gelu_erf(p.x), gelu_erf(p.y));
+      }
+      sg.end(tmap_out2, col0, row0, false);
+    }
+    shift8();
   }
 }
 
@@ -373,9 +358,7 @@
   static constexpr int B_BYTES = BN * BK * 2;
   static constexpr int STAGE_BYTES = A_BYTES + B_BYTES;
   static constexpr int STAGES = (BN == 256) ? 4 : (BN == 128 ? 6 : 8);
-  static constexpr int ACC_LD = BN + 4;
-  static constexpr int SMEM_BYTES = STAGES * STAGE_BYTES + 2 * kStageTileBytes + 1024  + 256 ;
-  static_assert(BM * ACC_LD * 4 <= STAGES * STAGE_BYTES, "the accumulator tile reuses the stage ring");
+  static constexpr int SMEM_BYTES = STAGES * STAGE_BYTES + kEpiGroups * kStageTileBytes + 1024  + 256 ;
   static_assert(SMEM_BYTES <= 232448, "exceeds 227 KB of shared memory per block");
 };
 
@@ -396,10 +379,8 @@
   extern __shared__ unsigned char smem_raw[];
   unsigned char* smem = reinterpret_cast<unsigned char*>((reinterpret_cast<uintptr_t>(smem_raw) + 1023) & ~uintptr_t(1023));
   unsigned char* staging = smem + STAGES * Cfg::STAGE_BYTES;
-  uint64_t* full_bar  = reinterpret_cast<uint64_t*>(staging + 2 * kStageTileBytes);
+  uint64_t* full_bar  = reinterpret_cast<uint64_t*>(staging + kEpiGroups * kStageTileBytes);
   uint64_t* empty_bar = full_bar + STAGES;
-  uint64_t* epi_bar   = empty_bar + STAGES;
-  float* acc_smem = reinterpret_cast<float*>(smem);
 
   const int warp = threadIdx.x >> 5, lane = threadIdx.x & 31;
   const uint32_t rank = CL == 2 ? cluster_ctarank() : 0u;
@@ -418,7 +399,6 @@
   }
   if (threadIdx.x == 32) {
     for (int s = 0; s < STAGES; ++s) { mbar_init(&full_bar[s], 1); mbar_init(&empty_bar[s], 8 * CL); }
-    mbar_init(epi_bar, 8 * CL);
     fence_mbar_init();
   }
   if constexpr (CL == 2) cluster_sync_all();
@@ -434,11 +414,9 @@
         if (hinted) tma_load_2d_hint(dst, tm, bar, c0, c1, pol);
         else        tma_load_2d(dst, tm, bar, c0, c1);
       };
-      int it = 0;
-      for (int tile = unit; tile < num_tiles; tile += num_units, ++it) {
+      for (int tile = unit; tile < num_tiles; tile += num_units) {
         int m_blk, n_blk;
         tile_coords(tile, num_m, num_n, group_m, m_blk, n_blk);
-        if (it > 0) mbar_wait(epi_bar, (uint32_t)(it - 1) & 1u);
         for (int kb = 0; kb < num_kb; ++kb) {
           mbar_wait(&empty_bar[stage], phase ^ 1);
           unsigned char* sa = smem + stage * Cfg::STAGE_BYTES;
@@ -468,7 +446,7 @@
   } else {
     asm volatile("setmaxnreg.inc.sync.aligned.u32 232;" ::: "memory");
     const int grp = (warp - 4) >> 2;
-    const int q = warp & 3;
+    EpiStage sg{staging + grp * kStageTileBytes, 1 + grp, (threadIdx.x & 127) == 0, 0};
     constexpr int TA = LAYOUT == 2 ? 1 : 0, TB = LAYOUT >= 1 ? 1 : 0;
     constexpr uint64_t a_step = TA ? 128 : 2, b_step = TB ? 128 : 2;
     const uint32_t a_off = (uint32_t)grp * 8192u;
@@ -502,29 +480,9 @@
         mbar_arrive(&empty_bar[prev]);
         if constexpr (CL == 2) mbar_arrive_remote(&empty_bar[prev], rank ^ 1u);
       }
-      named_bar_sync(3, 256);
-      {
-        const int r0 = grp * 64 + q * 16 + (lane >> 2);
-        float* p0 = acc_smem + (size_t)r0 * Cfg::ACC_LD + 2 * (lane & 3);
-        float* p1 = p0 + 8 * Cfg::ACC_LD;
-#pragma unroll
-        for (int j = 0; j < BN / 8; ++j) {
-          *reinterpret_cast<float2*>(p0 + 8 * j) = make_float2(acc[4 * j], acc[4 * j + 1]);
-          *reinterpret_cast<float2*>(p1 + 8 * j) = make_float2(acc[4 * j + 2], acc[4 * j + 3]);
-        }
-      }
-      named_bar_sync(3, 256);
-      const int row_in_tile = q * 32 + lane;
-      epilogue_drain_tile<BN, EPI>(ep, &tmap_out, &tmap_out2, staging, grp, acc_smem + (size_t)row_in_tile * Cfg::ACC_LD,
-                                   row_in_tile, (m_blk * CL + (int)rank) * BM, n_blk * BN);
-      fence_proxy_async();
-      __syncwarp();
-      if (lane == 0) {
-        mbar_arrive(epi_bar);
-        if constexpr (CL == 2) mbar_arrive_remote(epi_bar, rank ^ 1u);
-      }
-    }
-    if ((threadIdx.x & 127) == 0) bulk_wait<0>();
+      epilogue_tile<BN, EPI>(ep, &tmap_out, &tmap_out2, sg, acc, (m_blk * CL + (int)rank) * BM + grp * 64, n_blk * BN);
+    }
+    if (sg.issuer) bulk_wait<0>();
   }
   if constexpr (CL == 2) cluster_sync_all();
 }
@@ -736,7 +694,7 @@
   else             { if (int e = get_tmap(A, M, K, lda, 128, &ta)) return e; }
   if (layout >= 1) { if (int e = get_tmap(B, K, N, ldb, 64, &tb)) return e; }
   else             { if (int e = get_tmap(B, N, K, ldb, pair ? tile_n / 2 : tile_n, &tb)) return e; }
-  if (int e = get_tmap(out, M, N, ldo, 128, &to, out_f32)) return e;
+  if (int e = get_tmap(out, M, N, ldo, kBoxRows, &to, out_f32)) return e;
   DALM_REQUIRE(drop_p >= 0.f && drop_p < 1.f, "gemm: dropout p must be in [0,1)");
   GemmEpilogue ep = gemm_epilogue(M, N, K, tile_n, out, ldo, out_f32, resid, ldr, resid_f32);
   ep.bias = bias; ep.act = act; ep.alpha = alpha;
@@ -757,8 +715,8 @@
   CUtensorMap ta, tb, to, to2;
   if (int e = get_tmap(A, M, K, lda, 128, &ta)) return e;
   if (int e = get_tmap(B, N, K, ldb, 256, &tb)) return e;
-  if (int e = get_tmap(gu, M, N, ldgu, 128, &to, 0)) return e;
-  if (int e = get_tmap(act, M, N / 2, ldact, 128, &to2, 0)) return e;
+  if (int e = get_tmap(gu, M, N, ldgu, kBoxRows, &to, 0)) return e;
+  if (int e = get_tmap(act, M, N / 2, ldact, kBoxRows, &to2, 0)) return e;
   const GemmEpilogue ep = gemm_epilogue(M, N, K, 256, gu, ldgu);
   return launch_gemm<256, 0, Epi::SwiGLU>(ta, tb, to, ep, 0, (cudaStream_t)stream, &to2);
 }
@@ -772,8 +730,8 @@
   CUtensorMap ta, tb, to, to2;
   if (int e = get_tmap(A, M, K, lda, 128, &ta)) return e;
   if (int e = get_tmap(B, N, K, ldb, bn, &tb)) return e;
-  if (int e = get_tmap(pre, M, N, ldpre, 128, &to, 0)) return e;
-  if (int e = get_tmap(act, M, N, ldact, 128, &to2, 0)) return e;
+  if (int e = get_tmap(pre, M, N, ldpre, kBoxRows, &to, 0)) return e;
+  if (int e = get_tmap(act, M, N, ldact, kBoxRows, &to2, 0)) return e;
   GemmEpilogue ep = gemm_epilogue(M, N, K, bn, pre, ldpre);
   ep.bias = bias;
   return launch_gemm_bn<0, Epi::GeluPair>(bn, ta, tb, to, ep, 0, (cudaStream_t)stream, &to2);
@@ -790,7 +748,7 @@
   CUtensorMap ta, tb, to;
   if (int e = get_tmap(A, M, K, lda, 128, &ta)) return e;
   if (int e = get_tmap(B, N, K, ldb, 256, &tb)) return e;
-  if (int e = get_tmap(out, M, N, ldo, 128, &to, 0)) return e;
+  if (int e = get_tmap(out, M, N, ldo, kBoxRows, &to, 0)) return e;
   GemmEpilogue ep = gemm_epilogue(M, N, K, 256, out, ldo);
   ep.bias = bias;
   ep.rope_cos = cos_t; ep.rope_sin = sin_t; ep.rope_L = L; ep.rope_cols = rope_cols;
@@ -803,7 +761,7 @@
   CUtensorMap to2 = to;
   if (pre_out != nullptr) {
     DALM_REQUIRE(ld_pre >= rope_cols && (ld_pre % 8) == 0 && ((uintptr_t)pre_out & 15) == 0, "gemm_rope: pre_out leading dimension / alignment");
-    if (int e = get_tmap(pre_out, M, rope_cols, ld_pre, 128, &to2, 0)) return e;
+    if (int e = get_tmap(pre_out, M, rope_cols, ld_pre, kBoxRows, &to2, 0)) return e;
   }
   ep.q_norm = q_norm; ep.k_norm = k_norm; ep.nq_heads = nq_heads; ep.norm_eps = eps;
   ep.norm_rstd = rstd_out; ep.ld_rstd = ld_rstd; ep.norm_pre = pre_out != nullptr;
```

After: 73.55 (median of 6 runs). 1.04x the previous value.
